# AIRI-Institute/nablaDFT

Hardware: AMD Instinct MI355X
Metric: conformer-steps/sec (fwd+bwd) + MAE(E,F) vs CPU reference (higher is better)
Workload: dtype f32 (dense products >= 192 tiles: f32 values split exactly into 3 bf16 pieces, 6 MFMA piece products, f32 accumulate; non-finite operands give NaN where plain f32 gives inf); 1 GPU; PaiNN-OC (nablaDFT/painn_pyg, config/model/painn-oc.yaml: F=128 L=6 R=100 rc=5A K=100) energy+forces train step incl. neighbour list, L1+L2 loss, grad all-reduce, clip 5.0, AdamW lr 5e-4; synthetic ~42-atom drug-like conformers, 2048 conformers/GPU/step; conformers_per_gpu=2048, edges_last_step=1737976, parallelism=dp1

## Files before the change

nabladft_amd/csrc/edge.hip:

```cpp
#include "common.h"
#include <type_traits>
#include "lanes.h"

struct RbfArgs {
  const float4* geom; int E; int R; float inv_cutoff; float p, a, b, c; float coeff; const float* mu;
  float* rho; float* drho;
  int type;
  const float* theta;
  float norm_const;
  const float* grho;
  float* contrib;
};

__device__ __forceinline__ void rbf_envelope(const RbfArgs& q, float ds, float& env, float& denv) {
  env = 0.f; denv = 0.f;
  if (ds < 1.0f) {
    if (q.p > 0.f) {
      const float pm1 = powf(ds, q.p - 1.0f);
      const float p0 = pm1 * ds, p1 = p0 * ds, p2 = p1 * ds;
      env = 1.0f + q.a * p0 + q.b * p1 + q.c * p2;
      denv = q.a * q.p * pm1 + q.b * (q.p + 1.0f) * p0 + q.c * (q.p + 2.0f) * p1;
    } else {
      const float om = (1.0f - ds) * (1.0f + ds);
      env = expf(-(ds * ds) / om);
// ... 147 lines not shown
      const float* ps = q.PSI + (long)sp * F3;
      const float tpa = ps[f] * td, tpb = ps[F + f] * td, tpc = ps[2 * F + f] * td;
      const float* T = q.GTV + (long)k * F3;
      const float T0 = T[f], T1 = T[F + f], T2 = T[2 * F + f];
      const float gtma = q.GTX[(long)k * F + f];
      const float tmb = txb * pb + xb * tpb;
      gmb += T0 * tv0 + T1 * tv1 + T2 * tv2;
      const float gtmb = T0 * v0 + T1 * v1 + T2 * v2;
      gmc += T0 * tr0 + T1 * tr1 + T2 * tr2;
      const float gtmc = T0 * r0 + T1 * r1 + T2 * r2;
      gv0 += T0 * tmb; gv1 += T1 * tmb; gv2 += T2 * tmb;
      gtv0 += T0 * mb; gtv1 += T1 * mb; gtv2 += T2 * mb;
      gxa += gma * pa + gtma * tpa; gxb += gmb * pb + gtmb * tpb; gxc += gmc * pc + gtmc * tpc;
      gtxa += gtma * pa; gtxb += gtmb * pb; gtxc += gtmc * pc;
      float* gp = q.GPHI + (long)sp * F3;
      float* gs = q.GPSI + (long)sp * F3;
      const float ga = gma * xa + gtma * txa, gb = gmb * xb + gtmb * txb, gc = gmc * xc + gtmc * txc;
      gp[f] = ga; gp[F + f] = gb; gp[2 * F + f] = gc;
      sba += ga; sbb += gb; sbc += gc;
      gs[f] = gtma * xa * td; gs[F + f] = gtmb * xb * td; gs[2 * F + f] = gtmc * xc * td;
    } else {
      gxa += gma * pa; gxb += gmb * pb; gxc += gmc * pc;
      const float* ps = q.PSI + (long)sp * F3;
      float gd = gma * xa * ps[f] + gmb * xb * ps[F + f] + gmc * xc * ps[2 * F + f];
      float e0 = A0 * mc, e1 = A1 * mc, e2 = A2 * mc;
      gd = nq_wave_sum(gd); e0 = nq_wave_sum(e0); e1 = nq_wave_sum(e1); e2 = nq_wave_sum(e2);
      if (lane == 0) {
        float4* dstp = q.GEDGE + (long)wave * q.g.E + sp;
        float4 acc = *dstp;
        acc.x += gd; acc.y += e0; acc.z += e1; acc.w += e2;
        *dstp = acc;
      }
    }
  }
  q.GXH[o3 + f] = gxa; q.GXH[o3 + F + f] = gxb; q.GXH[o3 + 2 * F + f] = gxc;
  q.GV_out[o3 + f] = q.GV[o3 + f] + gv0;
  q.GV_out[o3 + F + f] = q.GV[o3 + F + f] + gv1;
  q.GV_out[o3 + 2 * F + f] = q.GV[o3 + 2 * F + f] + gv2;
  if (DUAL) {
    q.GTXH[o3 + f] = gtxa; q.GTXH[o3 + F + f] = gtxb; q.GTXH[o3 + 2 * F + f] = gtxc;
    q.GBR[o3 + f] = sba; q.GBR[o3 + F + f] = sbb; q.GBR[o3 + 2 * F + f] = sbc;
    q.GTV_out[o3 + f] = q.GTV[o3 + f] + gtv0;
    q.GTV_out[o3 + F + f] = q.GTV[o3 + F + f] + gtv1;
    q.GTV_out[o3 + 2 * F + f] = q.GTV[o3 + 2 * F + f] + gtv2;
  }
}


#define FUSED_THREADS 1024
#ifndef NQ_DUAL2_THREADS
#define NQ_DUAL2_THREADS 512
#endif
#ifndef NQ_TAN2_THREADS
#define NQ_TAN2_THREADS 768
#endif
#ifndef NQ_DUALNG2_THREADS
#define NQ_DUALNG2_THREADS 768
#endif
__host__ __device__ constexpr int fused_threads(int kind, int ch, bool l0 = false) {
  if (l0) return ch >= 4 ? 512 : 1024;
  return ch >= 4 ? 512
                 : (ch == 2 ? (kind == 3 ? NQ_DUAL2_THREADS : (kind == 4 ? NQ_DUALNG2_THREADS : (kind == 1 ? NQ_TAN2_THREADS : 1024)))
                            : (kind >= 3 ? 768 : 1024));
}
#define FUSED_THREADS_DUAL 1024

__device__ __forceinline__ float bcast_lane(float v, int t) {
  return __int_as_float(__builtin_amdgcn_readlane(__float_as_int(v), t));
}

#define RBFW_THREADS 256
__global__ __launch_bounds__(RBFW_THREADS) void k_rbf_window(const float4* __restrict__ geom, int E, FilterArgs fa, float* __restrict__ RW) {
  __shared__ float tile[RBFW_THREADS][RW_STRIDE + 1];
  const int e0 = blockIdx.x * RBFW_THREADS, e = e0 + threadIdx.x;
  if (e < E) {
    const int R = fa.R;
    const float dist = geom[e].w;
    const float ds = dist * fa.inv_cutoff;
    const int nwin = R < FWIN ? R : FWIN;
    int kc = (int)rintf(ds * (float)(R - 1));
    kc = min(max(kc, 0), R - 1);
    const int k0 = min(max(kc - FWIN / 2, 0), R - nwin);
    float beta = 1.f, dbeta = 0.f, env = 0.f, denv = 0.f;
    if (fa.mode == 0) {
      if (ds < 1.0f) {
        if (fa.p > 0.f) {
          const float pm1 = powf(ds, fa.p - 1.0f);
          const float p0 = pm1 * ds, p1 = p0 * ds, p2 = p1 * ds;
          env = 1.0f + fa.a * p0 + fa.b * p1 + fa.c * p2;
          denv = fa.a * fa.p * pm1 + fa.b * (fa.p + 1.0f) * p0 + fa.c * (fa.p + 2.0f) * p1;
        } else {
          const float om = (1.0f - ds) * (1.0f + ds);
          env = expf(-(ds * ds) / om);
          denv = -env * 2.0f * ds / (om * om);
        }
      }
    } else {
      const float arg = dist * (3.14159265358979323846f / fa.cutoff);
      const bool inside = dist < fa.cutoff;
      beta = inside ? 0.5f * (cosf(arg) + 1.0f) : 0.f;
      dbeta = inside ? -0.5f * (3.14159265358979323846f / fa.cutoff) * sinf(arg) : 0.f;
    }
    float* rw = tile[threadIdx.x];
#pragma unroll
    for (int t = 0; t < 16; ++t) {
      float rl = 0.f, drl = 0.f;
      if (t < nwin) {
        if (fa.mode == 0) {
          const float diff = ds - fa.mu[k0 + t];
          const float g = expf(fa.coeff * (diff * diff));
          rl = env * g;
          drl = fa.inv_cutoff * g * (denv + env * (2.0f * fa.coeff) * diff);
        } else {
          const float diff = dist - fa.mu[k0 + t];
          const float g = expf(fa.coeff * (diff * diff));
          if (fa.mode == 2) {
            rl = g;
            drl = g * (2.0f * fa.coeff) * diff;
          } else {
            rl = beta * g;
            drl = dbeta * g + beta * g * (2.0f * fa.coeff) * diff;
          }
        }
      }
      rw[t] = (t == 13) ? __int_as_float(k0) : (t == 14 ? beta : rl);
      rw[16 + t] = (t == 14) ? dbeta : drl;
    }
  }
  __syncthreads();
  const long base = (long)e0 * RW_STRIDE;
  const long lim = (long)min(RBFW_THREADS, E - e0) * RW_STRIDE;
#pragma unroll 4
  for (int i = threadIdx.x; i < RBFW_THREADS * RW_STRIDE; i += RBFW_THREADS)
    if (i < lim) RW[base + i] = tile[i / RW_STRIDE][i % RW_STRIDE];
}

struct RowRegs { int kk; float gx, gy, gz, td, t0, t1, t2, pf; };
#ifndef NQ_RW_TOUCH
#define NQ_RW_TOUCH 1
#endif
__device__ __forceinline__ void row_touch_done(const RowRegs& r) {
#if NQ_RW_TOUCH
  asm volatile("" ::"v"(r.pf));
#endif
}

template <bool NEED_T>
__device__ __forceinline__ void load_row(RowRegs& r, const NqGraphView& g, const float* __restrict__ TD, const float* __restrict__ TR,
                                         const float* __restrict__ RW, int sp0, int cnt, int lane) {
  r.kk = 0; r.gx = r.gy = r.gz = 0.f; r.td = r.t0 = r.t1 = r.t2 = 0.f; r.pf = 0.f;
  if (lane < cnt) {
    const int sp = sp0 + lane;
#if NQ_RW_TOUCH
    r.pf = RW[(long)sp * RW_STRIDE + 15];
#endif
    r.kk = g.col[sp];
    const float4 gm = g.geom[sp];
    r.gx = gm.x; r.gy = gm.y; r.gz = gm.z;
    if (NEED_T) { r.td = TD[sp]; r.t0 = TR[3 * (long)sp]; r.t1 = TR[3 * (long)sp + 1]; r.t2 = TR[3 * (long)sp + 2]; }
  }
}
template <bool PSI, int CH, int PM = 7, int QM = 7>
__device__ __forceinline__ void filter_eval(const WinRegs<PSI>& w, const float* wrt, int F, int F3, int fb, const float (&bra)[CH],
                                            const float (&brb)[CH], const float (&brc)[CH], float (&pa)[CH], float (&pb)[CH], float (&pc)[CH],
                                            float (&qa)[CH], float (&qb)[CH], float (&qc)[CH]) {
  typedef VOps<CH> O;
  typedef typename O::V V;
  constexpr int QMM = PSI ? QM : 0, TM = PM | QMM;
  constexpr bool PA = (PM & 1) != 0, PB = (PM & 2) != 0, PC = (PM & 4) != 0, QA = (QMM & 1) != 0, QB = (QMM & 2) != 0, QC = (QMM & 4) != 0;
  const V ba = O::from(bra), bb = O::from(brb), bc = O::from(brc);
  V va = O::splat(0.f), vb = va, vc = va, ua = va, ub = va, uc = va;
  if (PA) va = ba * O::splat(w.rr[14]);
  if (PB) vb = bb * O::splat(w.rr[14]);
  if (PC) vc = bc * O::splat(w.rr[14]);
  if (QA) ua = ba * O::splat(w.dd[14]);
  if (QB) ub = bb * O::splat(w.dd[14]);
  if (QC) uc = bc * O::splat(w.dd[14]);
  const int k0 = __builtin_amdgcn_readfirstlane(__float_as_int(w.rr[13]));
  const float* wk = wrt + k0 * F3 + fb;
#pragma unroll
  for (int t = 0; t < FWIN; ++t) {
    V wa = va, wb = va, wc = va;
    if (TM & 1) wa = lds_tap<CH>(wk + t * F3);
    if (TM & 2) wb = lds_tap<CH>(wk + t * F3 + F);
    if (TM & 4) wc = lds_tap<CH>(wk + t * F3 + 2 * F);
    if (PM) {
      const V r = O::splat(w.rr[t]);
      if (PA) va = O::fma(wa, r, va);
      if (PB) vb = O::fma(wb, r, vb);
      if (PC) vc = O::fma(wc, r, vc);
    }
    if (QMM) {
      const V d = O::splat(w.dd[t]);
      if (QA) ua = O::fma(wa, d, ua);
      if (QB) ub = O::fma(wb, d, ub);
      if (QC) uc = O::fma(wc, d, uc);
    }
  }
  O::to(pa, va); O::to(pb, vb); O::to(pc, vc);
  O::to(qa, ua); O::to(qb, ub); O::to(qc, uc);
}

#ifndef NQ_CLAIM_KINDS
#define NQ_CLAIM_KINDS 15
#endif
#ifndef NQ_CLAIM_ROWS
#define NQ_CLAIM_ROWS 1
#endif
#ifndef NQ_CLAIM_GROUPS_DUAL
#define NQ_CLAIM_GROUPS_DUAL 1
#endif
#ifndef NQ_CLAIM_GROUPS
// ... 31 lines not shown
  const int nxcd = (gridDim.x % (8 * nslices)) == 0 ? 8 : 1;                                   \
  const int bx = (int)(blockIdx.x / nxcd);                                                     \
  const int slice = bx % nslices, wg = bx / nslices;                                           \
  {                                 \
    const int Rp = fa.R < FWIN ? FWIN : fa.R;                                                  \
    const int per_row4 = (3 * FL) >> 2, fl4 = FL >> 2;                                         \
    float4* dst4 = reinterpret_cast<float4*>(wrt);                                             \
    for (int i = threadIdx.x; i < Rp * per_row4; i += blockDim.x) {                            \
      const int r = i / per_row4, c4 = i % per_row4, part = c4 / fl4, cc = c4 % fl4;           \
      dst4[i] = r < fa.R ? reinterpret_cast<const float4*>(fa.WRT + (long)r * F3 + part * F + slice * FL)[cc] : make_float4(0.f, 0.f, 0.f, 0.f); \
    }                                                                                          \
  }                                                                                            \
  __syncthreads();                                                                             \
  const int nslots = blockDim.x >> 6;                                                          \
  const int slot = __builtin_amdgcn_readfirstlane(threadIdx.x >> 6);                           \
  const int lane = threadIdx.x & 63;                                                           \
  const int lfb = lane * CH;                           \
  const int fb = slice * FL + lfb;                        \
  float bra[CH], brb[CH], brc[CH];                                                             \
  ldv<CH>(bra, fa.br + fb); ldv<CH>(brb, fa.br + F + fb); ldv<CH>(brc, fa.br + 2 * F + fb);    \
                                \
  const int per_x = (q.g.N + nxcd - 1) / nxcd;                                                 \
  const int x_lo = (int)(blockIdx.x % nxcd) * per_x, n_hi = min(q.g.N, x_lo + per_x);          \
  const int n_step = (int)(gridDim.x / nxcd / nslices) * nslots;                               \
                                                          \

template <bool TAN, int CH>
struct FwdOps { float xa[CH], xb[CH], xc[CH], va[CH], vb[CH], vc[CH], txa[CH], txb[CH], txc[CH], tva[CH], tvb[CH], tvc[CH]; };

template <bool TAN>
struct FwdSrc {
  __amdgpu_buffer_rsrc_t xh, v, txh, tv;
  __device__ __forceinline__ FwdSrc(const MsgArgs& q) : xh(row_rsrc(q.XH)), v(row_rsrc(q.V)), txh(row_rsrc(TAN ? q.TXH : q.XH)), tv(row_rsrc(TAN ? q.TV : q.V)) {}
};
template <bool TAN, int CH, bool L0 = false>
__device__ __forceinline__ void load_fwd(FwdOps<TAN, CH>& o, const FwdSrc<TAN>& src, int k, int F, int F3, int fb) {
  const int ob = fb * 4, r0 = k * F3 * 4, r1 = r0 + F * 4, r2 = r1 + F * 4;
  if (L0) {
    ldv_buf<CH>(o.xa, src.xh, ob, r0); ldv_buf<CH>(o.xc, src.xh, ob, r2);
    return;
  }
  ldv_buf<CH>(o.xa, src.xh, ob, r0); ldv_buf<CH>(o.xb, src.xh, ob, r1); ldv_buf<CH>(o.xc, src.xh, ob, r2);
  ldv_buf<CH>(o.va, src.v, ob, r0); ldv_buf<CH>(o.vb, src.v, ob, r1); ldv_buf<CH>(o.vc, src.v, ob, r2);
  if (TAN) {
    ldv_buf<CH>(o.txa, src.txh, ob, r0); ldv_buf<CH>(o.txb, src.txh, ob, r1); ldv_buf<CH>(o.txc, src.txh, ob, r2);
    ldv_buf<CH>(o.tva, src.tv, ob, r0); ldv_buf<CH>(o.tvb, src.tv, ob, r1); ldv_buf<CH>(o.tvc, src.tv, ob, r2);
  }
}

template <bool TAN, int CH, bool L0 = false>
__global__ __launch_bounds__(fused_threads(TAN ? 1 : 0, CH, L0)) void k_msgf_fwd(MsgArgs q, FilterArgs fa, const float* __restrict__ RW) {
  FUSED_PROLOGUE
  const FwdSrc<TAN> src(q);
  FUSED_ROWS(TAN ? 1 : 0) {
    const int beg = __builtin_amdgcn_readfirstlane(q.g.row_ptr[n]), end = __builtin_amdgcn_readfirstlane(q.g.row_ptr[n + 1]);
    float dx[CH], d0[CH], d1[CH], d2[CH];
#pragma unroll
    for (int c = 0; c < CH; ++c) dx[c] = d0[c] = d1[c] = d2[c] = 0.f;
    for (int c0 = beg; c0 < end; c0 += 64) {
      const int cnt = min(64, end - c0);
      RowRegs row;
      load_row<TAN>(row, q.g, q.TD, q.TR, RW, c0, cnt, lane);
      FwdOps<TAN, CH> opA, opB;
      load_fwd<TAN, CH, L0>(opA, src, bl_i(row.kk, 0), F, F3, fb);
      WinRegs<TAN> win;
      load_win<TAN>(win, RW, c0);
      auto step = [&](FwdOps<TAN, CH>& cur, FwdOps<TAN, CH>& nxt, int j, auto prefetch) __attribute__((always_inline)) {
        const int jn = min(j + 1, cnt - 1);
        if (decltype(prefetch)::value) load_fwd<TAN, CH, L0>(nxt, src, bl_i(row.kk, jn), F, F3, fb);
        float pa[CH], pb[CH], pc[CH], qa[CH], qb[CH], qc[CH];
        if (L0) filter_eval<TAN, CH, (TAN ? 4 : 5), 5>(win, wrt, FL, 3 * FL, lfb, bra, brb, brc, pa, pb, pc, qa, qb, qc);
        else filter_eval<TAN, CH>(win, wrt, FL, 3 * FL, lfb, bra, brb, brc, pa, pb, pc, qa, qb, qc);
        __builtin_amdgcn_sched_barrier(0);
        if (decltype(prefetch)::value) load_win<TAN>(win, RW, c0 + jn);
        const float gx = bl_f(row.gx, j), gy = bl_f(row.gy, j), gz = bl_f(row.gz, j);
        float td = 0.f, tr0 = 0.f, tr1 = 0.f, tr2 = 0.f;
        if (TAN) { td = bl_f(row.td, j); tr0 = bl_f(row.t0, j); tr1 = bl_f(row.t1, j); tr2 = bl_f(row.t2, j); }
#pragma unroll
        for (int c = 0; c < CH; ++c) {
          if (L0) {
            const float mc = cur.xc[c] * pc[c];
            if (!TAN) {
              const float m0 = mc * gx, m1 = mc * gy, m2 = mc * gz;
              dx[c] += cur.xa[c] * pa[c];
              d0[c] += m0; d1[c] += m1; d2[c] += m2;
            } else {
              const float tma = cur.xa[c] * (qa[c] * td), tmc = cur.xc[c] * (qc[c] * td);
              dx[c] += tma;
              d0[c] += fmaf(mc, tr0, tmc * gx);
              d1[c] += fmaf(mc, tr1, tmc * gy);
              d2[c] += fmaf(mc, tr2, tmc * gz);
            }
            continue;
          }
          const float mb = cur.xb[c] * pb[c], mc = cur.xc[c] * pc[c];
          if (!TAN) {
            dx[c] += cur.xa[c] * pa[c];
            d0[c] += cur.va[c] * mb + mc * gx;
            d1[c] += cur.vb[c] * mb + mc * gy;
            d2[c] += cur.vc[c] * mb + mc * gz;
          } else {
            const float tma = cur.txa[c] * pa[c] + cur.xa[c] * (qa[c] * td);
            const float tmb = cur.txb[c] * pb[c] + cur.xb[c] * (qb[c] * td);
            const float tmc = cur.txc[c] * pc[c] + cur.xc[c] * (qc[c] * td);
            dx[c] += tma;
            d0[c] += cur.tva[c] * mb + cur.va[c] * tmb + tmc * gx + mc * tr0;
            d1[c] += cur.tvb[c] * mb + cur.vb[c] * tmb + tmc * gy + mc * tr1;
            d2[c] += cur.tvc[c] * mb + cur.vc[c] * tmb + tmc * gz + mc * tr2;
          }
        }
      };
      const int pairs = cnt & ~1;
#pragma nounroll
      for (int j = 0; j < pairs; j += 2) {
        step(opA, opB, j, std::true_type());
        step(opB, opA, j + 1, std::true_type());
      }
      if (cnt & 1) step(opA, opB, cnt - 1, std::false_type());
      row_touch_done(row);
    }
    const long o = (long)n * F + fb, o3 = (long)n * F3 + fb;
    float x0[CH], w0[CH], w1[CH], w2[CH];
    if (L0) {
#pragma unroll
      for (int c = 0; c < CH; ++c) x0[c] = w0[c] = w1[c] = w2[c] = 0.f;
      if (!TAN) ldv<CH>(x0, q.X + o);
    } else if (!TAN) {
      ldv<CH>(x0, q.X + o); ldv<CH>(w0, q.V + o3); ldv<CH>(w1, q.V + o3 + F); ldv<CH>(w2, q.V + o3 + 2 * F);
    } else {
      ldv<CH>(x0, q.TX + o); ldv<CH>(w0, q.TV + o3); ldv<CH>(w1, q.TV + o3 + F); ldv<CH>(w2, q.TV + o3 + 2 * F);
    }
#pragma unroll
    for (int c = 0; c < CH; ++c) { x0[c] += dx[c]; w0[c] += d0[c]; w1[c] += d1[c]; w2[c] += d2[c]; }
    if (!TAN) {
      stv<CH>(q.XM + o, x0); stv<CH>(q.VM + o3, w0); stv<CH>(q.VM + o3 + F, w1); stv<CH>(q.VM + o3 + 2 * F, w2);
    } else {
      stv<CH>(q.TXM + o, x0); stv<CH>(q.TVM + o3, w0); stv<CH>(q.TVM + o3 + F, w1); stv<CH>(q.TVM + o3 + 2 * F, w2);
    }
  }
}

#ifndef NQ_ABLATE
#define NQ_ABLATE 0
#endif
#if NQ_ABLATE == 3
#define ABL_K(j) n
#else
#define ABL_K(j) bl_i(row.kk, j)
#endif
#if NQ_ABLATE == 4
#define ABL_SP(x) 0
#else
#define ABL_SP(x) (x)
#endif
template <bool DUAL, int CH>
struct RevOps { float A0[CH], A1[CH], A2[CH], gma[CH], T0[CH], T1[CH], T2[CH], gtma[CH]; };

template <bool DUAL>
struct RevSrc {
  __amdgpu_buffer_rsrc_t gv, gx, gtv, gtx;
  __device__ __forceinline__ RevSrc(const MsgRevArgs& q) : gv(row_rsrc(q.GV)), gx(row_rsrc(q.GX)), gtv(row_rsrc(DUAL ? q.GTV : q.GV)), gtx(row_rsrc(DUAL ? q.GTX : q.GX)) {}
};
template <bool DUAL, int CH>
__device__ __forceinline__ void load_rev(RevOps<DUAL, CH>& o, const RevSrc<DUAL>& src, int k, int F, int F3, int fb) {
  const int ob = fb * 4, r0 = k * F3 * 4, r1 = r0 + F * 4, r2 = r1 + F * 4, rx = k * F * 4;
  ldv_buf<CH>(o.A0, src.gv, ob, r0); ldv_buf<CH>(o.A1, src.gv, ob, r1); ldv_buf<CH>(o.A2, src.gv, ob, r2);
  ldv_buf<CH>(o.gma, src.gx, ob, rx);
  if (DUAL) {
    ldv_buf<CH>(o.T0, src.gtv, ob, r0); ldv_buf<CH>(o.T1, src.gtv, ob, r1); ldv_buf<CH>(o.T2, src.gtv, ob, r2);
    ldv_buf<CH>(o.gtma, src.gtx, ob, rx);
  }
}

#ifndef NQ_DUAL_NA_RESIDENT
#define NQ_DUAL_NA_RESIDENT 1
#endif
#ifndef NQ_DUAL_MIRROR
#define NQ_DUAL_MIRROR 1
#endif
#ifndef NQ_DUAL_KX_EARLY
#define NQ_DUAL_KX_EARLY 1
#endif
template <bool DUAL, int CH, bool GW, bool LITE = false, bool L0 = false>
__device__ __forceinline__ void msgf_rev_body(const MsgRevArgs& q, const FilterArgs& fa, const float* __restrict__ RW) {
  FUSED_PROLOGUE
  const RevSrc<DUAL> src(q);
  FUSED_ROWS(DUAL ? 3 : 2) {
    if (DUAL && q.row_filter) {
      const int mm = __builtin_amdgcn_readfirstlane(q.g.atom_mol[n]);
      const bool big = __builtin_amdgcn_readfirstlane(q.g.mol_ptr[mm + 1]) - __builtin_amdgcn_readfirstlane(q.g.mol_ptr[mm]) > q.mol_cap;
      if (big != (q.row_filter == 2)) continue;
    }
    const int beg = __builtin_amdgcn_readfirstlane(q.g.row_ptr[n]), end = __builtin_amdgcn_readfirstlane(q.g.row_ptr[n + 1]);
    const int nlow = (DUAL && GW) ? __builtin_amdgcn_readfirstlane(q.g.lowptr[n + 1]) - __builtin_amdgcn_readfirstlane(q.g.lowptr[n]) : 0;
    const long o3 = (long)n * F3 + fb;
    float xa[CH], xb[CH], xc[CH], v0[CH], v1[CH], v2[CH], txa[CH], txb[CH], txc[CH], tv0[CH], tv1[CH], tv2[CH];
    if (L0) {
#pragma unroll
      for (int c = 0; c < CH; ++c) xa[c] = xb[c] = xc[c] = v0[c] = v1[c] = v2[c] = 0.f;
      if (!DUAL) { ldv<CH>(xa, q.XH + o3); ldv<CH>(xc, q.XH + o3 + 2 * F); }
    } else {
      ldv<CH>(xa, q.XH + o3); ldv<CH>(xb, q.XH + o3 + F); ldv<CH>(xc, q.XH + o3 + 2 * F);
      ldv<CH>(v0, q.V + o3); ldv<CH>(v1, q.V + o3 + F); ldv<CH>(v2, q.V + o3 + 2 * F);
    }
    float nA0[CH], nA1[CH], nA2[CH], ngma[CH], nT0[CH], nT1[CH], nT2[CH], ngtma[CH];
    if (DUAL && !L0) {
      ldv<CH>(txa, q.TXH + o3); ldv<CH>(txb, q.TXH + o3 + F); ldv<CH>(txc, q.TXH + o3 + 2 * F);
      ldv<CH>(tv0, q.TV + o3); ldv<CH>(tv1, q.TV + o3 + F); ldv<CH>(tv2, q.TV + o3 + 2 * F);
#if NQ_DUAL_NA_RESIDENT
      if (GW) {
      ldv<CH>(nA0, q.GV + o3); ldv<CH>(nA1, q.GV + o3 + F); ldv<CH>(nA2, q.GV + o3 + 2 * F);
      ldv<CH>(nT0, q.GTV + o3); ldv<CH>(nT1, q.GTV + o3 + F); ldv<CH>(nT2, q.GTV + o3 + 2 * F);
      ldv<CH>(ngma, q.GX + (long)n * F + fb); ldv<CH>(ngtma, q.GTX + (long)n * F + fb);
      }
#endif
    } else {
#pragma unroll
      for (int c = 0; c < CH; ++c) txa[c] = txb[c] = txc[c] = tv0[c] = tv1[c] = tv2[c] = 0.f;
    }
    static_assert(!L0 || !GW, "the pair-row flavour has no layer-0 form");
    float gxa[CH], gxb[CH], gxc[CH], gv0[CH], gv1[CH], gv2[CH], gtxa[CH], gtxb[CH], gtxc[CH], gtv0[CH], gtv1[CH], gtv2[CH], sba[CH], sbb[CH], sbc[CH];
#pragma unroll
    for (int c = 0; c < CH; ++c) {
      gxa[c] = gxb[c] = gxc[c] = gv0[c] = gv1[c] = gv2[c] = 0.f;
      gtxa[c] = gtxb[c] = gtxc[c] = gtv0[c] = gtv1[c] = gtv2[c] = 0.f;
      sba[c] = sbb[c] = sbc[c] = 0.f;
    }
    for (int c0 = beg; c0 < end; c0 += 64) {
      const int cnt = min(64, end - c0);
      const int nlo = (DUAL && GW) ? max(0, min(cnt, nlow - (c0 - beg))) : 0;
      RowRegs row;
      load_row<DUAL>(row, q.g, q.TD, q.TR, RW, c0, cnt, lane);
      RevOps<DUAL, CH> opA, opB;
      load_rev<DUAL, CH>(opA, src, ABL_K(0), F, F3, fb);
      WinRegs<true> win;
      load_win<true>(win, RW, ABL_SP(c0));
      float4 eacc = make_float4(0.f, 0.f, 0.f, 0.f);
      auto step = [&](RevOps<DUAL, CH>& cur, RevOps<DUAL, CH>& nxt, int j, auto low_tag) __attribute__((always_inline)) {
        constexpr bool LOW = decltype(low_tag)::value;
        const int sp = c0 + j;
        const int jn = min(j + 1, cnt - 1);
        load_rev<DUAL, CH>(nxt, src, ABL_K(jn), F, F3, fb);
        float kxa[CH], kxb[CH], kxc[CH], kv0[CH], kv1[CH], kv2[CH], ktxa[CH], ktxb[CH], ktxc[CH], ktv0[CH], ktv1[CH], ktv2[CH];
        if (DUAL && GW && LOW && NQ_DUAL_KX_EARLY) {
          const long k3 = (long)ABL_K(j) * F3 + fb;
          ldv<CH>(kxa, q.XH + k3); ldv<CH>(kxb, q.XH + k3 + F); ldv<CH>(kxc, q.XH + k3 + 2 * F);
          ldv<CH>(kv0, q.V + k3); ldv<CH>(kv1, q.V + k3 + F); ldv<CH>(kv2, q.V + k3 + 2 * F);
          ldv<CH>(ktxa, q.TXH + k3); ldv<CH>(ktxb, q.TXH + k3 + F); ldv<CH>(ktxc, q.TXH + k3 + 2 * F);
          ldv<CH>(ktv0, q.TV + k3); ldv<CH>(ktv1, q.TV + k3 + F); ldv<CH>(ktv2, q.TV + k3 + 2 * F);
        }
        float pa[CH], pb[CH], pc[CH], qa[CH], qb[CH], qc[CH];
#if NQ_ABLATE == 2
#pragma unroll
        for (int c = 0; c < CH; ++c) { pa[c] = bra[c] * win.rr[0]; pb[c] = brb[c] * win.rr[1]; pc[c] = brc[c] * win.rr[2]; qa[c] = bra[c] * win.dd[0]; qb[c] = brb[c] * win.dd[1]; qc[c] = brc[c] * win.dd[2]; }
#else
        if (L0) filter_eval<true, CH, 5, 5>(win, wrt, FL, 3 * FL, lfb, bra, brb, brc, pa, pb, pc, qa, qb, qc);
        else filter_eval<true, CH>(win, wrt, FL, 3 * FL, lfb, bra, brb, brc, pa, pb, pc, qa, qb, qc);
#endif
        const float beta = win.rr[14], dbeta = win.dd[14];
        __builtin_amdgcn_sched_barrier(0);
        load_win<true>(win, RW, ABL_SP(c0 + jn));
        if (DUAL && GW && LOW && !NQ_DUAL_KX_EARLY) {
          const long k3 = (long)ABL_K(j) * F3 + fb;
          ldv<CH>(kxa, q.XH + k3); ldv<CH>(kxb, q.XH + k3 + F); ldv<CH>(kxc, q.XH + k3 + 2 * F);
          ldv<CH>(kv0, q.V + k3); ldv<CH>(kv1, q.V + k3 + F); ldv<CH>(kv2, q.V + k3 + 2 * F);
          ldv<CH>(ktxa, q.TXH + k3); ldv<CH>(ktxb, q.TXH + k3 + F); ldv<CH>(ktxc, q.TXH + k3 + 2 * F);
          ldv<CH>(ktv0, q.TV + k3); ldv<CH>(ktv1, q.TV + k3 + F); ldv<CH>(ktv2, q.TV + k3 + 2 * F);
        }
        const float r0 = -bl_f(row.gx, j), r1 = -bl_f(row.gy, j), r2 = -bl_f(row.gz, j);
        float td = 0.f, tr0 = 0.f, tr1 = 0.f, tr2 = 0.f;
        if (DUAL) { td = bl_f(row.td, j); tr0 = -bl_f(row.t0, j); tr1 = -bl_f(row.t1, j); tr2 = -bl_f(row.t2, j); }
        float gd = 0.f, e0 = 0.f, e1 = 0.f, e2 = 0.f;
        float ga[CH], gb[CH], gc[CH], ha[CH], hb[CH], hc[CH];
#pragma unroll
        for (int c = 0; c < CH; ++c) {
          const float A0 = cur.A0[c], A1 = cur.A1[c], A2 = cur.A2[c], gma = cur.gma[c];
          if (L0) {
            float gmc = A0 * r0 + A1 * r1 + A2 * r2;
            if (DUAL) {
              const float T0 = cur.T0[c], T1 = cur.T1[c], T2 = cur.T2[c], gtma = cur.gtma[c];
              gmc += T0 * tr0 + T1 * tr1 + T2 * tr2;
              const float gtmc = T0 * r0 + T1 * r1 + T2 * r2;
              gxa[c] += gma * pa[c] + gtma * (qa[c] * td); gxc[c] += gmc * pc[c] + gtmc * (qc[c] * td);
            } else {
              const float mc = xc[c] * pc[c];
              gxa[c] += gma * pa[c]; gxc[c] += gmc * pc[c];
              gd += fmaf(gmc * xc[c], qc[c], gma * xa[c] * qa[c]);
              e0 += A0 * mc; e1 += A1 * mc; e2 += A2 * mc;
            }
            continue;
          }
          const float mb = xb[c] * pb[c], mc = xc[c] * pc[c];
          float gmb = A0 * v0[c] + A1 * v1[c] + A2 * v2[c];
          float gmc = A0 * r0 + A1 * r1 + A2 * r2;
          gv0[c] += A0 * mb; gv1[c] += A1 * mb; gv2[c] += A2 * mb;
          if (DUAL) {
            const float tpa = qa[c] * td, tpb = qb[c] * td, tpc = qc[c] * td;
            const float T0 = cur.T0[c], T1 = cur.T1[c], T2 = cur.T2[c], gtma = cur.gtma[c];
            const float tmb = txb[c] * pb[c] + xb[c] * tpb;
            gmb += T0 * tv0[c] + T1 * tv1[c] + T2 * tv2[c];
            const float gtmb = T0 * v0[c] + T1 * v1[c] + T2 * v2[c];
            gmc += T0 * tr0 + T1 * tr1 + T2 * tr2;
            const float gtmc = T0 * r0 + T1 * r1 + T2 * r2;
            gv0[c] += T0 * tmb; gv1[c] += T1 * tmb; gv2[c] += T2 * tmb;
            if (!LITE) { gtv0[c] += T0 * mb; gtv1[c] += T1 * mb; gtv2[c] += T2 * mb; }
            gxa[c] += gma * pa[c] + gtma * tpa; gxb[c] += gmb * pb[c] + gtmb * tpb; gxc[c] += gmc * pc[c] + gtmc * tpc;
            if (!LITE) { gtxa[c] += gtma * pa[c]; gtxb[c] += gtmb * pb[c]; gtxc[c] += gtmc * pc[c]; }
            if (GW) {
              ga[c] = gma * xa[c] + gtma * txa[c]; gb[c] = gmb * xb[c] + gtmb * txb[c]; gc[c] = gmc * xc[c] + gtmc * txc[c];
              ha[c] = gtma * xa[c] * td; hb[c] = gtmb * xb[c] * td; hc[c] = gtmc * xc[c] * td;
              sba[c] += ga[c] * beta + ha[c] * dbeta;
              sbb[c] += gb[c] * beta + hb[c] * dbeta;
              sbc[c] += gc[c] * beta + hc[c] * dbeta;
            }
          } else {
            gxa[c] += gma * pa[c]; gxb[c] += gmb * pb[c]; gxc[c] += gmc * pc[c];
            gd += gma * xa[c] * qa[c] + gmb * xb[c] * qb[c] + gmc * xc[c] * qc[c];
            e0 += A0 * mc; e1 += A1 * mc; e2 += A2 * mc;
          }
        }
        if (DUAL && GW && LOW && NQ_ABLATE != 1) {
#if !NQ_DUAL_NA_RESIDENT
          __builtin_amdgcn_sched_barrier(0);
          ldv<CH>(nA0, q.GV + o3); ldv<CH>(nA1, q.GV + o3 + F); ldv<CH>(nA2, q.GV + o3 + 2 * F);
          ldv<CH>(nT0, q.GTV + o3); ldv<CH>(nT1, q.GTV + o3 + F); ldv<CH>(nT2, q.GTV + o3 + 2 * F);
          ldv<CH>(ngma, q.GX + (long)n * F + fb); ldv<CH>(ngtma, q.GTX + (long)n * F + fb);
#endif
#pragma unroll
          for (int c = 0; c < CH; ++c) {
            const float rgmb = nA0[c] * kv0[c] + nA1[c] * kv1[c] + nA2[c] * kv2[c] + (nT0[c] * ktv0[c] + nT1[c] * ktv1[c] + nT2[c] * ktv2[c]);
            const float rgtmb = nT0[c] * kv0[c] + nT1[c] * kv1[c] + nT2[c] * kv2[c];
            const float rgmc = -(nA0[c] * r0 + nA1[c] * r1 + nA2[c] * r2) - (nT0[c] * tr0 + nT1[c] * tr1 + nT2[c] * tr2);
            const float rgtmc = -(nT0[c] * r0 + nT1[c] * r1 + nT2[c] * r2);
            ga[c] += ngma[c] * kxa[c] + ngtma[c] * ktxa[c]; gb[c] += rgmb * kxb[c] + rgtmb * ktxb[c]; gc[c] += rgmc * kxc[c] + rgtmc * ktxc[c];
            ha[c] += ngtma[c] * kxa[c] * td; hb[c] += rgtmb * kxb[c] * td; hc[c] += rgtmc * kxc[c] * td;
          }
          float* gp = q.GPHI + (long)sp * F3 + fb;
          float* gs = q.GPSI + (long)sp * F3 + fb;
          stv_stream<CH>(gp, ga); stv_stream<CH>(gp + F, gb); stv_stream<CH>(gp + 2 * F, gc);
          stv_stream<CH>(gs, ha); stv_stream<CH>(gs + F, hb); stv_stream<CH>(gs + 2 * F, hc);
        } else if (!DUAL) {
          gd = nq_wave_sum(gd); e0 = nq_wave_sum(e0); e1 = nq_wave_sum(e1); e2 = nq_wave_sum(e2);
          const bool mine = lane == j;
          eacc.x = mine ? gd : eacc.x; eacc.y = mine ? e0 : eacc.y; eacc.z = mine ? e1 : eacc.z; eacc.w = mine ? e2 : eacc.w;
        }
      };
      int j = 0;
#pragma nounroll
      for (; j + 1 < nlo; j += 2) {
        step(opA, opB, j, std::true_type());
        step(opB, opA, j + 1, std::true_type());
      }
#if NQ_DUAL_MIRROR
      if (j < nlo) {
        step(opA, opB, j, std::true_type());
        ++j;
#pragma nounroll
        for (; j + 1 < cnt; j += 2) {
          step(opB, opA, j, std::false_type());
          step(opA, opB, j + 1, std::false_type());
        }
        if (j < cnt) step(opB, opA, j, std::false_type());
      } else {
#pragma nounroll
        for (; j + 1 < cnt; j += 2) {
          step(opA, opB, j, std::false_type());
          step(opB, opA, j + 1, std::false_type());
        }
        if (j < cnt) step(opA, opB, j, std::false_type());
      }
#else
      if (j < nlo) {
        step(opA, opB, j, std::true_type());
        ++j;
        opA = opB;
      }
#pragma nounroll
      for (; j + 1 < cnt; j += 2) {
        step(opA, opB, j, std::false_type());
        step(opB, opA, j + 1, std::false_type());
      }
      if (j < cnt) step(opA, opB, j, std::false_type());
#endif
      row_touch_done(row);
      if (!DUAL && lane < cnt) {
        float4* dstp = q.GEDGE + (long)slice * q.g.E + c0 + lane;
        float4 acc = *dstp;
        acc.x += eacc.x; acc.y += eacc.y; acc.z += eacc.z; acc.w += eacc.w;
        *dstp = acc;
      }
    }
    float g0[CH], g1[CH], g2[CH];
    stv<CH>(q.GXH + o3, gxa); stv<CH>(q.GXH + o3 + F, gxb); stv<CH>(q.GXH + o3 + 2 * F, gxc);
    if (L0) continue;
    ldv<CH>(g0, q.GV + o3); ldv<CH>(g1, q.GV + o3 + F); ldv<CH>(g2, q.GV + o3 + 2 * F);
#pragma unroll
    for (int c = 0; c < CH; ++c) { g0[c] += gv0[c]; g1[c] += gv1[c]; g2[c] += gv2[c]; }
    stv<CH>(q.GV_out + o3, g0); stv<CH>(q.GV_out + o3 + F, g1); stv<CH>(q.GV_out + o3 + 2 * F, g2);
    if (DUAL) {
      if (GW) { stv<CH>(q.GBR + o3, sba); stv<CH>(q.GBR + o3 + F, sbb); stv<CH>(q.GBR + o3 + 2 * F, sbc); }
      if (!LITE && !q.lite) {
        stv<CH>(q.GTXH + o3, gtxa); stv<CH>(q.GTXH + o3 + F, gtxb); stv<CH>(q.GTXH + o3 + 2 * F, gtxc);
        ldv<CH>(g0, q.GTV + o3); ldv<CH>(g1, q.GTV + o3 + F); ldv<CH>(g2, q.GTV + o3 + 2 * F);
#pragma unroll
        for (int c = 0; c < CH; ++c) { g0[c] += gtv0[c]; g1[c] += gtv1[c]; g2[c] += gtv2[c]; }
        stv<CH>(q.GTV_out + o3, g0); stv<CH>(q.GTV_out + o3 + F, g1); stv<CH>(q.GTV_out + o3 + 2 * F, g2);
      }
    }
  }
}


template <bool DUAL, int CH>
__global__ __launch_bounds__(fused_threads(DUAL ? 3 : 2, CH)) void k_msgf_rev(MsgRevArgs q, FilterArgs fa, const float* __restrict__ RW) {
  msgf_rev_body<DUAL, CH, DUAL>(q, fa, RW);
}
template <bool DUAL, int CH>
__global__ __launch_bounds__(fused_threads(DUAL ? 4 : 2, CH, true)) void k_msgf_rev_l0(MsgRevArgs q, FilterArgs fa, const float* __restrict__ RW) {
  msgf_rev_body<DUAL, CH, false, DUAL, true>(q, fa, RW);
}
template <bool LITE, int CH>
__global__ __launch_bounds__(fused_threads(4, CH)) void k_msgf_rev_nopair(MsgRevArgs q, FilterArgs fa, const float* __restrict__ RW) {
  msgf_rev_body<true, CH, false, LITE>(q, fa, RW);
}

#define SORT_CHUNK 256
struct K0Filter { const int* row_of; const int* col; const int* mol_ptr; const int* atom_mol; int cap; };
__device__ __forceinline__ int k0_key(const float* __restrict__ RW, int e, int E, const K0Filter& f) {
  if (e >= E) return -1;
  if (f.row_of && f.col[e] >= f.row_of[e]) return -1;
  if (f.cap > 0) { const int m = f.atom_mol[f.row_of[e]]; if (f.mol_ptr[m + 1] - f.mol_ptr[m] <= f.cap) return -1; }
  return __float_as_int(RW[(long)e * RW_STRIDE + 13]);
}
__global__ __launch_bounds__(SORT_CHUNK) void k_k0_hist(const float* __restrict__ RW, int E, int nbins, int* __restrict__ chunk_hist,
                                                        int* __restrict__ local_rank, K0Filter flt) {
  __shared__ int keys[SORT_CHUNK];
  __shared__ int hist[256];
  const int e = blockIdx.x * SORT_CHUNK + threadIdx.x;
  const int key = k0_key(RW, e, E, flt);
  keys[threadIdx.x] = key;
  if (threadIdx.x < nbins) hist[threadIdx.x] = 0;
  __syncthreads();
  if (key >= 0) {
    int r = 0;
    for (int i = 0; i < (int)threadIdx.x; ++i) r += (keys[i] == key);
    local_rank[e] = r;
    atomicAdd(&hist[key], 1);
  }
  __syncthreads();
  if (threadIdx.x < nbins) chunk_hist[(long)threadIdx.x * gridDim.x + blockIdx.x] = hist[threadIdx.x];
}
__global__ __launch_bounds__(256) void k_k0_scan(int* __restrict__ hist, int nchunks, int nbins, int* __restrict__ bin_total) {
  const int lane = threadIdx.x & 63;
  const int b = blockIdx.x * 4 + (threadIdx.x >> 6);
  if (b >= nbins) return;
  int* row = hist + (long)b * nchunks;
  int carry = 0;
  for (int c0 = 0; c0 < nchunks; c0 += 64) {
    const int c = c0 + lane;
    const int v = c < nchunks ? row[c] : 0;
    int sc = v;
#pragma unroll
    for (int off = 1; off < 64; off <<= 1) {
      const int t = __shfl_up(sc, off, 64);
      if (lane >= off) sc += t;
    }
    if (c < nchunks) row[c] = carry + sc - v;
    carry += __shfl(sc, 63, 64);
  }
  if (lane == 0) bin_total[b] = carry;
}
__global__ __launch_bounds__(SORT_CHUNK) void k_k0_scatter(const float* __restrict__ RW, int E, int nbins, const int* __restrict__ hist,
                                                           const int* __restrict__ bin_total, const int* __restrict__ local_rank,
                                                           int* __restrict__ order, K0Filter flt, int* __restrict__ count_out) {
  __shared__ int base[256];
// ... 303 lines not shown
  *lds = (size_t)(R < FWIN ? FWIN : R) * 3 * 64 * ch * sizeof(float);
  int per_cu = (int)((156 * 1024) / *lds);
  per_cu = per_cu < 1 ? 1 : (per_cu > 2 ? 2 : per_cu);
  int groups = 256 * per_cu / nslices;
  groups = groups < 8 ? 8 : (groups / 8) * 8;
  const int need = nq_cdiv(N, nslots);
  if (need < groups) groups = need;
  return groups * nslices;
}

#define FUSED_LAUNCH(KERN, Q, ...)                                                                                \
  do {                                                                                                            \
    NQ_DYN_LDS((KERN<__VA_ARGS__>), lds);                                                                         \
    hipLaunchKernelGGL((KERN<__VA_ARGS__>), dim3(grid), dim3(threads), lds, st, Q, fa, fa.RW);                    \
  } while (0)
#define FUSED_DISPATCH_CH(Q, LAUNCH1, LAUNCH2, LAUNCH4)                 \
  do {                                                                  \
    switch (ch) {                                                       \
      case 1: LAUNCH1; break;                                           \
      case 2: LAUNCH2; break;                                           \
      case 4: LAUNCH4; break;                                           \
      default: return nq_fail(NQ_ERR_ARG, "fused message kernels need hidden_channels in {64,128,256}"); \
    }                                                                   \
  } while (0)
#define FUSED_DISPATCH(KERN, FLAG, Q) FUSED_DISPATCH_CH(Q, FUSED_LAUNCH(KERN, Q, FLAG, 1), FUSED_LAUNCH(KERN, Q, FLAG, 2), FUSED_LAUNCH(KERN, Q, FLAG, 4))
#define FUSED_DISPATCH_FWD_L0(FLAG, Q) \
  FUSED_DISPATCH_CH(Q, FUSED_LAUNCH(k_msgf_fwd, Q, FLAG, 1, true), FUSED_LAUNCH(k_msgf_fwd, Q, FLAG, 2, true), FUSED_LAUNCH(k_msgf_fwd, Q, FLAG, 4, true))

int nq_msgf_fwd(hipStream_t st, const MsgArgs& q, const FilterArgs& fa, bool tangent, bool layer0) {
  NQ_PROF(st, tangent ? (layer0 ? "msgf_tan_l0" : "msgf_tan") : (layer0 ? "msgf_fwd_l0" : "msgf_fwd"));
  if (q.g.N <= 0) return NQ_OK;
  if ((size_t)q.g.N * 3 * q.F * 4 >= 0xfffff000ull) return nq_fail(NQ_ERR_ARG, "fused message kernels: a node array of %d atoms x %d channels exceeds the 4 GB a buffer descriptor's scalar offset reaches", q.g.N, 3 * q.F);
  int threads; size_t lds;
  const int ch = fused_ch(tangent ? 1 : 0, q.F, q.g.N);
  const int grid = fused_grid(q.g.N, q.F, ch, &threads, &lds, fa.R, fused_threads(tangent ? 1 : 0, ch, layer0));
  if (layer0 && tangent) FUSED_DISPATCH_FWD_L0(true, q);
  else if (layer0) FUSED_DISPATCH_FWD_L0(false, q);
  else if (tangent) FUSED_DISPATCH(k_msgf_fwd, true, q);
  else FUSED_DISPATCH(k_msgf_fwd, false, q);
  NQ_LAUNCH_CHECK();
  return NQ_OK;
}

int nq_force_planes(int F, int N, bool fused) { return fused ? F / (64 * fused_ch(2, F, N)) : F / 64; }

int nq_msgf_rev(hipStream_t st, const MsgRevArgs& q, const FilterArgs& fa, bool dual, bool pair_rows, bool layer0) {
  layer0 = layer0 && (!dual || (!pair_rows && q.lite));
  NQ_PROF(st, dual ? (pair_rows ? "msgf_rev_dual" : (layer0 ? "msgf_rev_dual_ng_l0" : "msgf_rev_dual_ng")) : (layer0 ? "msgf_rev_force_l0" : "msgf_rev_force"));
  if (q.g.N <= 0) return NQ_OK;
  if ((size_t)q.g.N * 3 * q.F * 4 >= 0xfffff000ull) return nq_fail(NQ_ERR_ARG, "fused message kernels: a node array of %d atoms x %d channels exceeds the 4 GB a buffer descriptor's scalar offset reaches", q.g.N, 3 * q.F);
  int threads; size_t lds;
  const int kind = dual ? (pair_rows ? 3 : 4) : 2;
  const int ch = fused_ch(dual ? 3 : 2, q.F, q.g.N);
  const int grid = fused_grid(q.g.N, q.F, ch, &threads, &lds, fa.R, fused_threads(kind, ch, layer0));
  if (layer0 && dual) FUSED_DISPATCH(k_msgf_rev_l0, true, q);
  else if (layer0) FUSED_DISPATCH(k_msgf_rev_l0, false, q);
  else if (dual && !pair_rows && q.lite) FUSED_DISPATCH(k_msgf_rev_nopair, true, q);
  else if (dual && !pair_rows) FUSED_DISPATCH(k_msgf_rev_nopair, false, q);
  else if (dual) FUSED_DISPATCH(k_msgf_rev, true, q);
  else FUSED_DISPATCH(k_msgf_rev, false, q);
  NQ_LAUNCH_CHECK();
  return NQ_OK;
}

static int gwr_nbins(int R) { return R - (R < FWIN ? R : FWIN) + 1; }
static int gwr_chunks(int E) {
  int chunk_len = nq_cdiv(E, GWR_CHUNKS);
  if (chunk_len < 64) chunk_len = 64;
  return nq_cdiv(E, chunk_len);
}
size_t nq_k0_sort_scratch_ints(int E, int R) { return (size_t)nq_cdiv(E, SORT_CHUNK) * gwr_nbins(R) + (size_t)E + 256; }
int nq_k0_sort(hipStream_t st, const float* RW, int E, int R, int* order, int* scratch, const int* row_of, const int* col, const int* mol_ptr,
               const int* atom_mol, int cap, int* count_out) {
  NQ_PROF(st, "k0_sort");
  K0Filter flt{row_of, col, mol_ptr, atom_mol, (row_of && mol_ptr && atom_mol) ? cap : 0};
  const int nbins = gwr_nbins(R), nchunks = nq_cdiv(E, SORT_CHUNK);
  if (nbins > 256) return nq_fail(NQ_ERR_ARG, "k0 sort supports at most 256 bins (num_rbf <= 268)");
  int* chunk_hist = scratch; int* local_rank = scratch + (size_t)nchunks * nbins; int* bin_total = local_rank + E;
  hipLaunchKernelGGL(k_k0_hist, dim3(nchunks), dim3(SORT_CHUNK), 0, st, RW, E, nbins, chunk_hist, local_rank, flt);
  NQ_LAUNCH_CHECK();
  hipLaunchKernelGGL(k_k0_scan, dim3(nq_cdiv(nbins, 4)), dim3(256), 0, st, chunk_hist, nchunks, nbins, bin_total);
  NQ_LAUNCH_CHECK();
  hipLaunchKernelGGL(k_k0_scatter, dim3(nchunks), dim3(SORT_CHUNK), 0, st, RW, E, nbins, chunk_hist, bin_total, local_rank, order, flt, count_out);
  NQ_LAUNCH_CHECK();
  return NQ_OK;
}

size_t nq_gwr_scratch_floats(int E, int F, int R, int parts) { const size_t nc = gwr_chunks(E); return nc * R * parts * F + 2 * nc + 16; }

int nq_gwr_sorted(hipStream_t st, const float* GPHI, const float* GPSI, const float* RW, const int* order, int E, int F, int R, float* gWr,
                  float* scratch, int parts, const int* count_dev) {
  NQ_PROF(st, "gwr_sorted");
  const int nchunks = gwr_chunks(E), chunk_len = nq_cdiv(E, nchunks);
  float* part = scratch;
  const int F3 = parts * F;
  int* chunk_range = reinterpret_cast<int*>(scratch + (size_t)nchunks * R * F3);
  dim3 grid(nq_cdiv(nchunks, GWR_WAVES), parts);
  switch (F / 64) {
    case 1: hipLaunchKernelGGL((k_gwr_sorted<1>), grid, dim3(GWR_WAVES * 64), 0, st, GPHI, GPSI, RW, order, E, F, F3, R, chunk_len, part, chunk_range, count_dev); break;
    case 2: hipLaunchKernelGGL((k_gwr_sorted<2>), grid, dim3(GWR_WAVES * 64), 0, st, GPHI, GPSI, RW, order, E, F, F3, R, chunk_len, part, chunk_range, count_dev); break;
    case 4: hipLaunchKernelGGL((k_gwr_sorted<4>), grid, dim3(GWR_WAVES * 64), 0, st, GPHI, GPSI, RW, order, E, F, F3, R, chunk_len, part, chunk_range, count_dev); break;
    default: return nq_fail(NQ_ERR_ARG, "gwr_sorted needs hidden_channels in {64,128,256}");
  }
  NQ_LAUNCH_CHECK();
  hipLaunchKernelGGL(k_gwr_reduce, dim3(nq_cdiv((long)R * F3, 256)), dim3(256), 0, st, part, chunk_range, nq_cdiv(E, chunk_len), R, F3, gWr);
  NQ_LAUNCH_CHECK();
  return NQ_OK;
// ... 2 lines not shown
```

Measured before the change: 52460 conformer-steps/s.

## Use single operand set with late reload to raise block size in tangent/dual kernels

For the tangent forward and lite non-pair dual reverse message kernels at CH=2, the double-buffered operand sets (opA/opB) are replaced by a single set that is reloaded at the end of each step after a scheduling barrier. Base pointers are pinned into VGPRs via inline asm. Block size goes from 768 to 1024 threads for these kernels. This cuts register pressure so more waves fit per CU, but it loses the overlap between the next neighbour's loads and the current filter math.

```diff
diff --git a/nabladft_amd/csrc/edge.hip b/nabladft_amd/csrc/edge.hip
--- a/nabladft_amd/csrc/edge.hip
+++ b/nabladft_amd/csrc/edge.hip
@@ -223,15 +223,22 @@
 #define NQ_DUAL2_THREADS 512
 #endif
 #ifndef NQ_TAN2_THREADS
-#define NQ_TAN2_THREADS 768
+#define NQ_TAN2_THREADS 1024
 #endif
 #ifndef NQ_DUALNG2_THREADS
 #define NQ_DUALNG2_THREADS 768
 #endif
-__host__ __device__ constexpr int fused_threads(int kind, int ch, bool l0 = false) {
+#ifndef NQ_DUALNG2_LITE_THREADS
+#define NQ_DUALNG2_LITE_THREADS 1024
+#endif
+__host__ __device__ constexpr bool fused_one_set(int kind, int ch, bool l0 = false, bool lite = false) {
+  return !l0 && ch == 2 && (kind == 1 || (kind == 4 && lite));
+}
+__host__ __device__ constexpr int fused_threads(int kind, int ch, bool l0 = false, bool lite = false) {
   if (l0) return ch >= 4 ? 512 : 1024;
+  if (fused_one_set(kind, ch, l0, lite)) return kind == 1 ? NQ_TAN2_THREADS : NQ_DUALNG2_LITE_THREADS;
   return ch >= 4 ? 512
-                 : (ch == 2 ? (kind == 3 ? NQ_DUAL2_THREADS : (kind == 4 ? NQ_DUALNG2_THREADS : (kind == 1 ? NQ_TAN2_THREADS : 1024)))
+                 : (ch == 2 ? (kind == 3 ? NQ_DUAL2_THREADS : (kind == 4 ? NQ_DUALNG2_THREADS : 1024))
                             : (kind >= 3 ? 768 : 1024));
 }
 #define FUSED_THREADS_DUAL 1024
@@ -316,19 +323,29 @@
 #endif
 }
 
+template <bool PIN, class T>
+__device__ __forceinline__ T* vgpr_base(T* p) {
+  if (PIN) asm volatile("" : "+v"(p));
+  return p;
+}
+struct RowSrc { const int* col; const float4* geom; const float* TD; const float* TR; };
+template <bool PIN, bool NEED_T>
+__device__ __forceinline__ RowSrc row_src(const NqGraphView& g, const float* TD, const float* TR) {
+  return RowSrc{vgpr_base<PIN>(g.col), vgpr_base<PIN>(g.geom), NEED_T ? vgpr_base<PIN>(TD) : nullptr, NEED_T ? vgpr_base<PIN>(TR) : nullptr};
+}
+
 template <bool NEED_T>
-__device__ __forceinline__ void load_row(RowRegs& r, const NqGraphView& g, const float* __restrict__ TD, const float* __restrict__ TR,
-                                         const float* __restrict__ RW, int sp0, int cnt, int lane) {
+__device__ __forceinline__ void load_row(RowRegs& r, const RowSrc& s, const float* __restrict__ RW, int sp0, int cnt, int lane) {
   r.kk = 0; r.gx = r.gy = r.gz = 0.f; r.td = r.t0 = r.t1 = r.t2 = 0.f; r.pf = 0.f;
   if (lane < cnt) {
     const int sp = sp0 + lane;
 #if NQ_RW_TOUCH
     r.pf = RW[(long)sp * RW_STRIDE + 15];
 #endif
-    r.kk = g.col[sp];
-    const float4 gm = g.geom[sp];
+    r.kk = s.col[sp];
+    const float4 gm = s.geom[sp];
     r.gx = gm.x; r.gy = gm.y; r.gz = gm.z;
-    if (NEED_T) { r.td = TD[sp]; r.t0 = TR[3 * (long)sp]; r.t1 = TR[3 * (long)sp + 1]; r.t2 = TR[3 * (long)sp + 2]; }
+    if (NEED_T) { r.td = s.TD[sp]; r.t0 = s.TR[3 * (long)sp]; r.t1 = s.TR[3 * (long)sp + 1]; r.t2 = s.TR[3 * (long)sp + 2]; }
   }
 }
 template <bool PSI, int CH, int PM = 7, int QM = 7>
@@ -466,6 +483,10 @@
 __global__ __launch_bounds__(fused_threads(TAN ? 1 : 0, CH, L0)) void k_msgf_fwd(MsgArgs q, FilterArgs fa, const float* __restrict__ RW) {
   FUSED_PROLOGUE
   const FwdSrc<TAN> src(q);
+  constexpr bool ONE_SET = fused_one_set(TAN ? 1 : 0, CH, L0);
+  const RowSrc rsrc = row_src<ONE_SET, TAN>(q.g, q.TD, q.TR);
+  const float* const own_tx = vgpr_base<ONE_SET>(q.TX), * const own_tv = vgpr_base<ONE_SET>(q.TV);
+  float* const out_tx = vgpr_base<ONE_SET>(q.TXM), * const out_tv = vgpr_base<ONE_SET>(q.TVM);
   FUSED_ROWS(TAN ? 1 : 0) {
     const int beg = __builtin_amdgcn_readfirstlane(q.g.row_ptr[n]), end = __builtin_amdgcn_readfirstlane(q.g.row_ptr[n + 1]);
     float dx[CH], d0[CH], d1[CH], d2[CH];
@@ -474,14 +495,14 @@
     for (int c0 = beg; c0 < end; c0 += 64) {
       const int cnt = min(64, end - c0);
       RowRegs row;
-      load_row<TAN>(row, q.g, q.TD, q.TR, RW, c0, cnt, lane);
+      load_row<TAN>(row, rsrc, RW, c0, cnt, lane);
       FwdOps<TAN, CH> opA, opB;
       load_fwd<TAN, CH, L0>(opA, src, bl_i(row.kk, 0), F, F3, fb);
       WinRegs<TAN> win;
       load_win<TAN>(win, RW, c0);
       auto step = [&](FwdOps<TAN, CH>& cur, FwdOps<TAN, CH>& nxt, int j, auto prefetch) __attribute__((always_inline)) {
         const int jn = min(j + 1, cnt - 1);
-        if (decltype(prefetch)::value) load_fwd<TAN, CH, L0>(nxt, src, bl_i(row.kk, jn), F, F3, fb);
+        if (!ONE_SET && decltype(prefetch)::value) load_fwd<TAN, CH, L0>(nxt, src, bl_i(row.kk, jn), F, F3, fb);
         float pa[CH], pb[CH], pc[CH], qa[CH], qb[CH], qc[CH];
         if (L0) filter_eval<TAN, CH, (TAN ? 4 : 5), 5>(win, wrt, FL, 3 * FL, lfb, bra, brb, brc, pa, pb, pc, qa, qb, qc);
         else filter_eval<TAN, CH>(win, wrt, FL, 3 * FL, lfb, bra, brb, brc, pa, pb, pc, qa, qb, qc);
@@ -523,14 +544,24 @@
             d2[c] += cur.tvc[c] * mb + cur.vc[c] * tmb + tmc * gz + mc * tr2;
           }
         }
+        if (ONE_SET && decltype(prefetch)::value) {
+          __builtin_amdgcn_sched_barrier(0);
+          load_fwd<TAN, CH, L0>(cur, src, bl_i(row.kk, jn), F, F3, fb);
+        }
       };
-      const int pairs = cnt & ~1;
+      if (ONE_SET) {
 #pragma nounroll
-      for (int j = 0; j < pairs; j += 2) {
-        step(opA, opB, j, std::true_type());
-        step(opB, opA, j + 1, std::true_type());
+        for (int j = 0; j < cnt - 1; ++j) step(opA, opA, j, std::true_type());
+        step(opA, opA, cnt - 1, std::false_type());
+      } else {
+        const int pairs = cnt & ~1;
+#pragma nounroll
+        for (int j = 0; j < pairs; j += 2) {
+          step(opA, opB, j, std::true_type());
+          step(opB, opA, j + 1, std::true_type());
+        }
+        if (cnt & 1) step(opA, opB, cnt - 1, std::false_type());
       }
-      if (cnt & 1) step(opA, opB, cnt - 1, std::false_type());
       row_touch_done(row);
     }
     const long o = (long)n * F + fb, o3 = (long)n * F3 + fb;
@@ -542,14 +573,14 @@
     } else if (!TAN) {
       ldv<CH>(x0, q.X + o); ldv<CH>(w0, q.V + o3); ldv<CH>(w1, q.V + o3 + F); ldv<CH>(w2, q.V + o3 + 2 * F);
     } else {
-      ldv<CH>(x0, q.TX + o); ldv<CH>(w0, q.TV + o3); ldv<CH>(w1, q.TV + o3 + F); ldv<CH>(w2, q.TV + o3 + 2 * F);
+      ldv<CH>(x0, own_tx + o); ldv<CH>(w0, own_tv + o3); ldv<CH>(w1, own_tv + o3 + F); ldv<CH>(w2, own_tv + o3 + 2 * F);
     }
 #pragma unroll
     for (int c = 0; c < CH; ++c) { x0[c] += dx[c]; w0[c] += d0[c]; w1[c] += d1[c]; w2[c] += d2[c]; }
     if (!TAN) {
       stv<CH>(q.XM + o, x0); stv<CH>(q.VM + o3, w0); stv<CH>(q.VM + o3 + F, w1); stv<CH>(q.VM + o3 + 2 * F, w2);
     } else {
-      stv<CH>(q.TXM + o, x0); stv<CH>(q.TVM + o3, w0); stv<CH>(q.TVM + o3 + F, w1); stv<CH>(q.TVM + o3 + 2 * F, w2);
+      stv<CH>(out_tx + o, x0); stv<CH>(out_tv + o3, w0); stv<CH>(out_tv + o3 + F, w1); stv<CH>(out_tv + o3 + 2 * F, w2);
     }
   }
 }
@@ -599,6 +630,8 @@
 __device__ __forceinline__ void msgf_rev_body(const MsgRevArgs& q, const FilterArgs& fa, const float* __restrict__ RW) {
   FUSED_PROLOGUE
   const RevSrc<DUAL> src(q);
+  constexpr bool ONE_SET = fused_one_set(DUAL ? (GW ? 3 : 4) : 2, CH, L0, LITE);
+  const RowSrc rsrc = row_src<ONE_SET, DUAL>(q.g, q.TD, q.TR);
   FUSED_ROWS(DUAL ? 3 : 2) {
     if (DUAL && q.row_filter) {
       const int mm = __builtin_amdgcn_readfirstlane(q.g.atom_mol[n]);
@@ -644,7 +677,7 @@
       const int cnt = min(64, end - c0);
       const int nlo = (DUAL && GW) ? max(0, min(cnt, nlow - (c0 - beg))) : 0;
       RowRegs row;
-      load_row<DUAL>(row, q.g, q.TD, q.TR, RW, c0, cnt, lane);
+      load_row<DUAL>(row, rsrc, RW, c0, cnt, lane);
       RevOps<DUAL, CH> opA, opB;
       load_rev<DUAL, CH>(opA, src, ABL_K(0), F, F3, fb);
       WinRegs<true> win;
@@ -654,7 +687,7 @@
         constexpr bool LOW = decltype(low_tag)::value;
         const int sp = c0 + j;
         const int jn = min(j + 1, cnt - 1);
-        load_rev<DUAL, CH>(nxt, src, ABL_K(jn), F, F3, fb);
+        if (!ONE_SET) load_rev<DUAL, CH>(nxt, src, ABL_K(jn), F, F3, fb);
         float kxa[CH], kxb[CH], kxc[CH], kv0[CH], kv1[CH], kv2[CH], ktxa[CH], ktxb[CH], ktxc[CH], ktv0[CH], ktv1[CH], ktv2[CH];
         if (DUAL && GW && LOW && NQ_DUAL_KX_EARLY) {
           const long k3 = (long)ABL_K(j) * F3 + fb;
@@ -733,6 +766,10 @@
             e0 += A0 * mc; e1 += A1 * mc; e2 += A2 * mc;
           }
         }
+        if (ONE_SET) {
+          __builtin_amdgcn_sched_barrier(0);
+          load_rev<DUAL, CH>(cur, src, ABL_K(jn), F, F3, fb);
+        }
         if (DUAL && GW && LOW && NQ_ABLATE != 1) {
 #if !NQ_DUAL_NA_RESIDENT
           __builtin_amdgcn_sched_barrier(0);
@@ -760,42 +797,47 @@
         }
       };
       int j = 0;
+      if (ONE_SET) {
 #pragma nounroll
-      for (; j + 1 < nlo; j += 2) {
-        step(opA, opB, j, std::true_type());
-        step(opB, opA, j + 1, std::true_type());
-      }
+        for (; j < cnt; ++j) step(opA, opA, j, std::false_type());
+      } else {
+#pragma nounroll
+        for (; j + 1 < nlo; j += 2) {
+          step(opA, opB, j, std::true_type());
+          step(opB, opA, j + 1, std::true_type());
+        }
 #if NQ_DUAL_MIRROR
-      if (j < nlo) {
-        step(opA, opB, j, std::true_type());
-        ++j;
+        if (j < nlo) {
+          step(opA, opB, j, std::true_type());
+          ++j;
 #pragma nounroll
-        for (; j + 1 < cnt; j += 2) {
-          step(opB, opA, j, std::false_type());
-          step(opA, opB, j + 1, std::false_type());
-        }
-        if (j < cnt) step(opB, opA, j, std::false_type());
-      } else {
+          for (; j + 1 < cnt; j += 2) {
+            step(opB, opA, j, std::false_type());
+            step(opA, opB, j + 1, std::false_type());
+          }
+          if (j < cnt) step(opB, opA, j, std::false_type());
+        } else {
+#pragma nounroll
+          for (; j + 1 < cnt; j += 2) {
+            step(opA, opB, j, std::false_type());
+            step(opB, opA, j + 1, std::false_type());
+          }
+          if (j < cnt) step(opA, opB, j, std::false_type());
+        }
+#else
+        if (j < nlo) {
+          step(opA, opB, j, std::true_type());
+          ++j;
+          opA = opB;
+        }
 #pragma nounroll
         for (; j + 1 < cnt; j += 2) {
           step(opA, opB, j, std::false_type());
           step(opB, opA, j + 1, std::false_type());
         }
         if (j < cnt) step(opA, opB, j, std::false_type());
+#endif
       }
-#else
-      if (j < nlo) {
-        step(opA, opB, j, std::true_type());
-        ++j;
-        opA = opB;
-      }
-#pragma nounroll
-      for (; j + 1 < cnt; j += 2) {
-        step(opA, opB, j, std::false_type());
-        step(opB, opA, j + 1, std::false_type());
-      }
-      if (j < cnt) step(opA, opB, j, std::false_type());
-#endif
       row_touch_done(row);
       if (!DUAL && lane < cnt) {
         float4* dstp = q.GEDGE + (long)slice * q.g.E + c0 + lane;
@@ -834,7 +876,7 @@
   msgf_rev_body<DUAL, CH, false, DUAL, true>(q, fa, RW);
 }
 template <bool LITE, int CH>
-__global__ __launch_bounds__(fused_threads(4, CH)) void k_msgf_rev_nopair(MsgRevArgs q, FilterArgs fa, const float* __restrict__ RW) {
+__global__ __launch_bounds__(fused_threads(4, CH, false, LITE)) void k_msgf_rev_nopair(MsgRevArgs q, FilterArgs fa, const float* __restrict__ RW) {
   msgf_rev_body<true, CH, false, LITE>(q, fa, RW);
 }
 
@@ -1244,7 +1286,7 @@
   int threads; size_t lds;
   const int kind = dual ? (pair_rows ? 3 : 4) : 2;
   const int ch = fused_ch(dual ? 3 : 2, q.F, q.g.N);
-  const int grid = fused_grid(q.g.N, q.F, ch, &threads, &lds, fa.R, fused_threads(kind, ch, layer0));
+  const int grid = fused_grid(q.g.N, q.F, ch, &threads, &lds, fa.R, fused_threads(kind, ch, layer0, q.lite));
   if (layer0 && dual) FUSED_DISPATCH(k_msgf_rev_l0, true, q);
   else if (layer0) FUSED_DISPATCH(k_msgf_rev_l0, false, q);
   else if (dual && !pair_rows && q.lite) FUSED_DISPATCH(k_msgf_rev_nopair, true, q);
```

After: 52870 conformer-steps/s (median of 6 runs). No clear change (+0.8%).
